# avik-pal/LocalRegNeuralDE.jl

Measured on NVIDIA B200. Metric: mnist_ode_train_samples_per_s, higher is better.
Workload: dtype tf32x3

## Files before the change

localregneuralde.jl_b200/csrc/lrnde_adjoint.cu:

```cuda
#include "lrnde_adjoint.h"

#include <stdio.h>
#include <stdlib.h>
#include <string.h>

#include <algorithm>

#include "lrnde_fused_dev.cuh"

enum {
  LA_ALPHA = 0,
  LA_S1 = 2,
  LA_DEL = 8,
  LA_CC = 13,
  LA_HH = 18,
  LA_EPS = 23,
  LA_DBT = 29,
  LA_HBB = 30,
  LA_HBT = 31,
  LA_NARR = 32
};

#ifdef LRNDE_UMMA_TRACE
__device__ long long g_adj_trace[1024];
// ... 586 lines not shown
            }
          } else if (g < 4) {
            r = __ldcg(reinterpret_cast<const float4*>(o.Q0 + (size_t)b * LR_ZROW + c4 * 4));
          } else if (o.Q1) {
            r = __ldcg(reinterpret_cast<const float4*>(o.Q1 + (size_t)b * LR_ZROW + c4 * 4));
          }
        }
        dst[g] = r;
      }
    };
    if (niter > 0) load_iter(0, v[0]);
    if (niter > 1) load_iter(1, v[1]);
    for (int it0 = 0; it0 < niter; it0 += 2) {
#pragma unroll
      for (int dd = 0; dd < 2; ++dd) {
        const int it = it0 + dd;
        if (it < niter) {
          const int s = it % NS, ph = (it / NS) & 1;
          uint8_t* stage = smem + (size_t)s * kPaStageBytes;
          const Ops o = ops_of(it);
          mbar_wait(&empty_bar[s], (uint32_t)(ph ^ 1));
#pragma unroll
          for (int g = 0; g < 6; ++g) {
            const int li = tid + (g & 1) * PT;
            const int bl = li >> 5, c4 = li & 31;
            const int grp = c4 >> 3, c32 = (c4 & 7) >> 1, half = c4 & 1, k4 = bl >> 2, r = bl & 3;
            const uint32_t off = (uint32_t)((k4 * 4 + grp) * 512 + r * 128 + ((c32 ^ r) << 5) + half * 16);
            float4 xv = (g >= 4 && !o.Q1) ? v[dd][g - 2] : v[dd][g];
            const float sc = (g < 2) ? 1.0f : ((g < 4) ? o.s0 : o.s1);
            xv.x *= sc; xv.y *= sc; xv.z *= sc; xv.w *= sc;
            float4 hi, lo;
            if (q.passes == 3) {
              hi = make_float4(tf32_rna(xv.x), tf32_rna(xv.y), tf32_rna(xv.z), tf32_rna(xv.w));
              lo = make_float4(tf32_rna(xv.x - hi.x), tf32_rna(xv.y - hi.y), tf32_rna(xv.z - hi.z), tf32_rna(xv.w - hi.w));
            } else { hi = xv; lo = make_float4(0.f, 0.f, 0.f, 0.f); }
            uint8_t* img = stage + (g >> 1) * 32768;
            *reinterpret_cast<float4*>(img + off) = hi;
            *reinterpret_cast<float4*>(img + 16384 + off) = lo;
          }
          if (it + 2 < niter) load_iter(it + 2, v[dd]);
          fence_proxy_async();
          __syncwarp();
          if (lane == 0) mbar_arrive(&full_bar[s]);
        }
      }
    }
    mbar_wait(&done_bar, 0);
    tc_fence_after();
    const int quarter = (warp & 3) * 32;
    const int wgroup = (warp - 2) >> 2;
    const int mrow = quarter + lane;
    const int nacc = (job == 0) ? 4 : 2;
    float* out;
    if (job == 0) out = q.partP + (size_t)split * 4 * 16384;
    else out = (job == 1 ? q.partX : q.partL) + ((size_t)split * q.ntile + tile) * 2 * 16384;
    for (int a = 0; a < nacc; ++a) {
      for (int cb = wgroup; cb < 8; cb += kEpiWarps / 4) {
        float r[16];
        tmem_ld16(tmem_base + ((uint32_t)quarter << 16) + (uint32_t)(a * 128 + cb * 16), r);
        float4* o4 = reinterpret_cast<float4*>(out + (size_t)a * 16384 + (size_t)mrow * 128 + cb * 16);
        if (niter == 0) {
#pragma unroll
          for (int j = 0; j < 16; ++j) r[j] = 0.0f;
        }
#pragma unroll
        for (int j = 0; j < 4; ++j) o4[j] = make_float4(r[4 * j], r[4 * j + 1], r[4 * j + 2], r[4 * j + 3]);
      }
    }
    tc_fence_before();
  }
  __syncthreads();
  if (warp == 1) {
    tc_fence_after();
    asm volatile("tcgen05.dealloc.cta_group::1.sync.aligned.b32 %0, %1;" ::"r"(tmem_base), "r"(512u) : "memory");
  }
}

struct AReduceP {
  SolveDev* S;
  const float* partP; const float* partX; const float* partL;
  float* RP; float* RX; float* RL;
  int nP, nD, ntile;
};
__global__ void __launch_bounds__(256) adj_reduce_kernel(AReduceP p) {
  if (p.S->done) return;
  const size_t nP4 = 4 * 4096, nX4 = (size_t)p.ntile * 2 * 4096;
  for (size_t i = blockIdx.x * (size_t)blockDim.x + threadIdx.x; i < nP4 + 2 * nX4; i += (size_t)gridDim.x * blockDim.x) {
    float4 s = make_float4(0.f, 0.f, 0.f, 0.f);
    if (i < nP4) {
      const float4* src = reinterpret_cast<const float4*>(p.partP) + i;
#pragma unroll 8
      for (int k = 0; k < p.nP; ++k) {
        const float4 v = __ldcg(src + (size_t)k * nP4);
        s.x += v.x; s.y += v.y; s.z += v.z; s.w += v.w;
      }
      reinterpret_cast<float4*>(p.RP)[i] = s;
    } else {
      const bool isx = (i - nP4) < nX4;
      const size_t j = isx ? (i - nP4) : (i - nP4 - nX4);
      const float4* src = reinterpret_cast<const float4*>(isx ? p.partX : p.partL) + j;
      for (int k = 0; k < p.nD; ++k) {
        const float4 v = __ldcg(src + (size_t)k * nX4);
        s.x += v.x; s.y += v.y; s.z += v.z; s.w += v.w;
      }
      const size_t tile = j / (2 * 4096), rem = j % (2 * 4096), vv = rem / 4096, mn = rem % 4096;
      float4* dst = reinterpret_cast<float4*>(isx ? p.RX : p.RL);
      dst[(vv * p.ntile + tile) * 4096 + mn] = s;
    }
  }
}

struct AMuP {
  SolveDev* S;
  const float* RP; const float* RX; const float* RL;
  const float* W2a;
  const float* W1T;
  int D, H, td, Kaug, ntile;
  long w1_off, w2_off;
  long nparams;
};
__global__ void __launch_bounds__(512) adj_mu_kernel(AMuP p) {
  SolveDev* S = p.S;
  if (S->done) return;
  const int slot = S->slot, next = (S->slot + 1) % S->cap;
  const float* mu_n = lr_slot_u(S, slot) + S->lam_len;
  float* mu_new = lr_slot_u(S, next) + S->lam_len;
  const float dt = S->err.scale, abstol = S->abstol, reltol = S->reltol;
  const int H = p.H, D = p.D, Kaug = p.Kaug;
  const long n1 = (long)H * (D + p.td + 1), n2 = (long)D * Kaug;
  const size_t RXs = (size_t)p.ntile * 128 * 128;
  const bool multi = S->reduce_mu && S->nranks > 1;
  const int par = (int)(S->mseq & 1ull);
  float* st0 = multi ? lr_mbox_stage(S->mbox[S->rank], par, 0) : nullptr;
  float* st1 = multi ? lr_mbox_stage(S->mbox[S->rank], par, 1) : nullptr;
  double acc = 0.0;
  for (long i = blockIdx.x * (long)blockDim.x + threadIdx.x; i < n1 + n2; i += (long)gridDim.x * blockDim.x) {
    float g0, g1;
    long pidx;
    if (i < n1) {
      const int d = (int)(i / H), r = (int)(i % H);
      pidx = p.w1_off + i;
      if (d < D) {
        float a0 = p.RX[(size_t)d * 128 + r], a1 = p.RX[RXs + (size_t)d * 128 + r];
        const float* w = p.W2a + d;
        const float* P0 = p.RP + r;
        const float* P1 = p.RP + 16384 + r;
#pragma unroll 8
        for (int k = 0; k < Kaug; ++k) {
          const float wv = __ldg(w + (size_t)k * D);
          a0 = fmaf(P0[k * 128], wv, a0);
          a1 = fmaf(P1[k * 128], wv, a1);
        }
        g0 = a0; g1 = a1;
      } else {
        const int krow = (p.td && d == D) ? Kaug : Kaug + 1;
        g0 = p.RP[(size_t)krow * 128 + r];
        g1 = p.RP[16384 + (size_t)krow * 128 + r];
      }
    } else {
      const long i2 = i - n1;
      const int k = (int)(i2 / D), d = (int)(i2 % D);
      pidx = p.w2_off + i2;
      float a0 = 0.0f, a1 = 0.0f;
      const float* P0 = p.RP + 2 * 16384 + (size_t)k * 128;
      const float* P1 = p.RP + 3 * 16384 + (size_t)k * 128;
      const float* w = p.W1T + d;
#pragma unroll 8
      for (int r = 0; r < H; ++r) {
        const float wv = __ldg(w + (size_t)r * D);
        a0 = fmaf(P0[r], wv, a0);
        a1 = fmaf(P1[r], wv, a1);
      }
      g0 = fmaf(-dt, a0, p.RL[(size_t)d * 128 + k]);
      g1 = fmaf(-dt, a1, p.RL[RXs + (size_t)d * 128 + k]);
    }
    if (multi) {
      st0[pidx] = g0;
      st1[pidx] = g1;
      continue;
    }
    const float mn = mu_n[pidx];
    const float mv = fmaf(-dt, g0, mn);
    mu_new[pidx] = mv;
    const float ut = -dt * g1;
    const float r = ut / (abstol + fmaxf(fabsf(mn), fabsf(mv)) * reltol);
    acc += (double)(r * r);
  }
  if (multi) {
    __threadfence_system();
    __syncthreads();
    if (threadIdx.x == 0) {
      const unsigned int prev = atomicAdd(S->mucounter, 1u);
      if (prev == gridDim.x - 1) {
        *S->mucounter = 0;
        __threadfence_system();
        for (int r = 0; r < S->nranks; ++r) {
          volatile unsigned long long* f = &S->mbox[r]->mflag[par][S->rank];
          *f = S->mseq + 1;
        }
      }
    }
    return;
  }
  __shared__ double sh[16];
  for (int o = 16; o > 0; o >>= 1) acc += __shfl_down_sync(0xffffffffu, acc, o);
  if ((threadIdx.x & 31) == 0) sh[threadIdx.x >> 5] = acc;
  __syncthreads();
  if (threadIdx.x == 0) {
    double s = 0.0;
    for (int w = 0; w < (int)(blockDim.x >> 5); ++w) s += sh[w];
    S->partials[LR_ERR_BLOCKS + blockIdx.x] = s;
  }
}

__global__ void __launch_bounds__(256) adj_mu_finish_kernel(SolveDev* S) {
  if (S->done) return;
  const int par = (int)(S->mseq & 1ull);
  LrMailbox* mine = S->mbox[S->rank];
  if (threadIdx.x == 0) {
    long long spins = 0;
    for (int r = 0; r < S->nranks; ++r) {
      volatile unsigned long long* f = &mine->mflag[par][r];
      while (*f != S->mseq + 1) {
        __nanosleep(40);
        if (++spins > (1ll << 26)) { lr_peer_timeout(S); break; }
      }
    }
    __threadfence_system();
  }
  __syncthreads();
  const int slot = S->slot, next = (S->slot + 1) % S->cap;
  const size_t P = S->mu_len;
  const float* mu_n = lr_slot_u(S, slot) + S->lam_len;
  float* mu_new = lr_slot_u(S, next) + S->lam_len;
  const float* mg_n = S->muglob + (size_t)slot * P;
  float* mg_new = S->muglob + (size_t)next * P;
  const float* own0 = lr_mbox_stage(mine, par, 0);
  const float dt = S->err.scale, abstol = S->abstol, reltol = S->reltol;
  double acc = 0.0;
  for (size_t i = blockIdx.x * (size_t)blockDim.x + threadIdx.x; i < P; i += (size_t)gridDim.x * blockDim.x) {
    float g0 = 0.0f, g1 = 0.0f;
    for (int r = 0; r < S->nranks; ++r) {
      g0 += ((const volatile float*)lr_mbox_stage(S->mbox[r], par, 0))[i];
      g1 += ((const volatile float*)lr_mbox_stage(S->mbox[r], par, 1))[i];
    }
    mu_new[i] = fmaf(-dt, ((const volatile float*)own0)[i], mu_n[i]);
    const float mn = mg_n[i];
    const float mv = fmaf(-dt, g0, mn);
    mg_new[i] = mv;
    const float ut = -dt * g1;
    const float rr = ut / (abstol + fmaxf(fabsf(mn), fabsf(mv)) * reltol);
    acc += (double)(rr * rr);
  }
  __shared__ double sh[8];
  for (int o = 16; o > 0; o >>= 1) acc += __shfl_down_sync(0xffffffffu, acc, o);
  if ((threadIdx.x & 31) == 0) sh[threadIdx.x >> 5] = acc;
  __syncthreads();
  if (threadIdx.x == 0) {
    double s = 0.0;
    for (int w = 0; w < 8; ++w) s += sh[w];
    S->partials[LR_ERR_BLOCKS + blockIdx.x] = s;
  }
}

}

#define LRA_COUNT(ctx) do { if ((ctx)->capturing) (ctx)->captured++; else (ctx)->launches++; } while (0)

bool LatentAdjoint::eligible(const lrnde_model* m) {
  FusedShape s;
  if (!lrf_shape(m, &s)) return false;
  return s.KS <= 14 && s.Kaug + 2 <= 128;
}

LatentAdjoint::LatentAdjoint(lrnde_ctx* c, const lrnde_model* mm, const float* p, int64_t b, int npasses)
    : ctx(c), m(mm), ps(p), B(b), passes(npasses) {
  lrf_shape(m, &sh);
  ntiles = (int)((B + fused::kNT - 1) / fused::kNT);
  zlen = (size_t)LR_ZROW * (size_t)ntiles * fused::kNT;
  nunits = (int)((B + 15) / 16);
  unit_bytes = (size_t)sh.nfull * 8192 + (size_t)sh.ntail * 2048;
  const int maxc = std::max(1, 148 / sh.n_mt);
  const int rounds = (nunits + maxc - 1) / maxc;
  nclusters = (nunits + rounds - 1) / rounds;
  ntile_d = (sh.D + 127) / 128;
  const int nchunk_tot = (int)((B + 31) / 32);
  const double wP = 13.0, wD = 2.0 * ntile_d;
  int wantP = std::max(1, (int)(148.0 * wP / (wP + wD)));
  int cP = std::max(1, (nchunk_tot + wantP - 1) / wantP);
  chunkP = cP * 32;
  nP = (int)((B + chunkP - 1) / chunkP);
  int wantD = std::max(1, (148 - nP) / (2 * ntile_d));
  int cD = std::max(1, (nchunk_tot + wantD - 1) / wantD);
  chunkD = cD * 32;
  nD = (int)((B + chunkD - 1) / chunkD);
  Mz = (float*)ctx->alloc(sizeof(float) * 128 * 128);
  ws = (float*)ctx->alloc(sizeof(float) * LA_NARR * zlen);
  alpha_in = (float*)ctx->alloc(sizeof(float) * zlen);
  hbuf = (float*)ctx->alloc((size_t)ntiles * 4 * unit_bytes);
  partP = (float*)ctx->alloc(sizeof(float) * (size_t)nP * 4 * 16384);
  partX = (float*)ctx->alloc(sizeof(float) * (size_t)nD * ntile_d * 2 * 16384);
  partL = (float*)ctx->alloc(sizeof(float) * (size_t)nD * ntile_d * 2 * 16384);
  RP = (float*)ctx->alloc(sizeof(float) * 4 * 16384);
  RX = (float*)ctx->alloc(sizeof(float) * (size_t)ntile_d * 2 * 16384);
  RL = (float*)ctx->alloc(sizeof(float) * (size_t)ntile_d * 2 * 16384);
  static bool attr_set = false;
  if (!attr_set) {
    constexpr int kChainSmem = 4 * (3 * 8192 + 3 * 2048) + ladj::kTapeBufs * ladj::kTapeBufBytes + 1024;
    LR_CUDA(cudaFuncSetAttribute(ladj::adj_chain_kernel<ACT_IDENTITY, false>, cudaFuncAttributeMaxDynamicSharedMemorySize, kChainSmem));
    LR_CUDA(cudaFuncSetAttribute(ladj::adj_chain_kernel<ACT_IDENTITY, true>, cudaFuncAttributeMaxDynamicSharedMemorySize, kChainSmem));
    LR_CUDA(cudaFuncSetAttribute(ladj::adj_chain_kernel<ACT_TANH, false>, cudaFuncAttributeMaxDynamicSharedMemorySize, kChainSmem));
    LR_CUDA(cudaFuncSetAttribute(ladj::adj_chain_kernel<ACT_TANH, true>, cudaFuncAttributeMaxDynamicSharedMemorySize, kChainSmem));
    LR_CUDA(cudaFuncSetAttribute(ladj::adj_chain_kernel<ACT_GELU, false>, cudaFuncAttributeMaxDynamicSharedMemorySize, kChainSmem));
    LR_CUDA(cudaFuncSetAttribute(ladj::adj_chain_kernel<ACT_GELU, true>, cudaFuncAttributeMaxDynamicSharedMemorySize, kChainSmem));
    LR_CUDA(cudaFuncSetAttribute(ladj::adj_chain_kernel<ACT_SIGMOID, false>, cudaFuncAttributeMaxDynamicSharedMemorySize, kChainSmem));
    LR_CUDA(cudaFuncSetAttribute(ladj::adj_chain_kernel<ACT_SIGMOID, true>, cudaFuncAttributeMaxDynamicSharedMemorySize, kChainSmem));
    LR_CUDA(cudaFuncSetAttribute(ladj::adj_chain_kernel<ACT_RELU, false>, cudaFuncAttributeMaxDynamicSharedMemorySize, kChainSmem));
    LR_CUDA(cudaFuncSetAttribute(ladj::adj_chain_kernel<ACT_RELU, true>, cudaFuncAttributeMaxDynamicSharedMemorySize, kChainSmem));
    LR_CUDA(cudaFuncSetAttribute(ladj::pairacc_kernel, cudaFuncAttributeMaxDynamicSharedMemorySize, ladj::pairacc_smem()));
    attr_set = true;
  }
  if (getenv("LRNDE_FUSED_VERBOSE"))
    fprintf(stderr, "[lrnde adjoint] B=%lld tiles=%d units=%d kgemm clusters=%d pairacc: nP=%d x %d samples, nD=%d x %d samples x %d tiles\n",
            (long long)B, ntiles, nunits, nclusters, nP, chunkP, nD, chunkD, ntile_d);
}

LatentAdjoint::~LatentAdjoint() {
  ctx->release(Mz); ctx->release(ws); ctx->release(alpha_in); ctx->release(hbuf);
  ctx->release(partP); ctx->release(partX); ctx->release(partL);
  ctx->release(RP); ctx->release(RX); ctx->release(RL);
}

void LatentAdjoint::prepare(const float* mz_plain) {
  if (mz_plain) { Mz_ext = mz_plain; return; }
  lrf_mz_plain(ctx, m, ps, Mz);
  LRA_COUNT(ctx);
}

static void lra_launch_chain(LatentAdjoint& E, SolveDev* S, int single) {
  const FusedShape& sh = E.sh;
  const LayerInfo& L1 = E.m->layers[0];
  ladj::AChainP cp;
  memset(&cp, 0, sizeof(cp));
  cp.S = S; cp.single = single; cp.Mz = E.Mz_ext ? E.Mz_ext : E.Mz;
  cp.w1t = sh.td ? E.ps + L1.w_off + (size_t)sh.D * sh.H : nullptr;
  cp.b1 = E.ps + L1.b_off;
  cp.Zx = E.Zx; cp.alpha_in = E.alpha_in; cp.ws = E.ws; cp.zlen = E.zlen;
  cp.hbuf = E.hbuf; cp.unit_bytes = (uint32_t)E.unit_bytes;
  cp.B = (int)E.B; cp.H = sh.H; cp.td = sh.td; cp.Kaug = sh.Kaug; cp.KS = sh.KS; cp.nfull = sh.nfull; cp.ntail = sh.ntail;
  cp.passes = E.passes;
  const size_t smem_c = 4 * ((size_t)sh.nfull * 8192 + (size_t)sh.ntail * 2048) + ladj::kTapeBufs * ladj::kTapeBufBytes + 1024;
  cudaStream_t st = E.ctx->stream;
#define LRA_CHAIN(A) do { if (single) ladj::adj_chain_kernel<A, true><<<E.ntiles, fused::kThreads, smem_c, st>>>(cp); \
                         else ladj::adj_chain_kernel<A, false><<<E.ntiles, fused::kThreads, smem_c, st>>>(cp); } while (0)
  switch (sh.act) {
    case ACT_TANH: LRA_CHAIN(ACT_TANH); break;
    case ACT_GELU: LRA_CHAIN(ACT_GELU); break;
    case ACT_SIGMOID: LRA_CHAIN(ACT_SIGMOID); break;
    case ACT_RELU: LRA_CHAIN(ACT_RELU); break;
    default: LRA_CHAIN(ACT_IDENTITY); break;
  }
#undef LRA_CHAIN
  LRA_COUNT(E.ctx);
  LR_CUDA(cudaGetLastError());
}

static void lra_launch_pairacc(LatentAdjoint& E, SolveDev* S) {
  ladj::PairAccP q;
  memset(&q, 0, sizeof(q));
  q.S = S; q.ws = E.ws; q.zlen = E.zlen; q.x = E.x; q.D = E.sh.D; q.B = (int)E.B;
  q.nP = E.nP; q.chunkP = E.chunkP; q.nD = E.nD; q.chunkD = E.chunkD; q.ntile = E.ntile_d;
  q.partP = E.partP; q.partX = E.partX; q.partL = E.partL; q.passes = E.passes;
  int n = 0;
  for (int j = 1; j <= 7; ++j) {
    const float bj = (j <= 6) ? lr_tsit5_a(5, j - 1) : 0.0f;
    const float btj = lr_tsit5_btilde(j - 1);
    const int del = (j == 1) ? -1 : ((j == 7) ? -10 : LA_DEL + j - 2);
    const int hh = (j == 1) ? -2 : ((j == 7) ? -11 : LA_HH + j - 2);
    const int cc = (j == 1) ? -3 : ((j == 7) ? -12 : LA_CC + j - 2);
    q.term[n++] = {cc, del, bj, btj, 0};
    if (j >= 2) q.term[n++] = {hh, LA_EPS + j - 2, bj, btj, 1};
  }
  q.nterm = n;
  const int grid = E.nP + 2 * E.ntile_d * E.nD;
  ladj::pairacc_kernel<<<grid, fused::kThreads, ladj::pairacc_smem(), E.ctx->stream>>>(q);
  LRA_COUNT(E.ctx);
  LR_CUDA(cudaGetLastError());
}

static void lra_launch_mu(LatentAdjoint& E, SolveDev* S) {
  cudaStream_t st = E.ctx->stream;
  ladj::AReduceP r;
  r.S = S; r.partP = E.partP; r.partX = E.partX; r.partL = E.partL; r.RP = E.RP; r.RX = E.RX; r.RL = E.RL;
  r.nP = E.nP; r.nD = E.nD; r.ntile = E.ntile_d;
  const size_t n4 = 4 * 4096 + 2 * (size_t)E.ntile_d * 2 * 4096;
  ladj::adj_reduce_kernel<<<(int)((n4 + 255) / 256), 256, 0, st>>>(r);
  LRA_COUNT(E.ctx);
  const LayerInfo& L1 = E.m->layers[0];
  const LayerInfo& L2 = E.m->layers[1];
  ladj::AMuP mp;
  memset(&mp, 0, sizeof(mp));
  mp.S = S; mp.RP = E.RP; mp.RX = E.RX; mp.RL = E.RL;
  mp.W2a = E.ps + L2.w_off; mp.W1T = E.W1T;
  mp.D = E.sh.D; mp.H = E.sh.H; mp.td = E.sh.td; mp.Kaug = E.sh.Kaug; mp.ntile = E.ntile_d;
  mp.w1_off = (long)L1.w_off; mp.w2_off = (long)L2.w_off; mp.nparams = (long)E.m->nparams;
  ladj::adj_mu_kernel<<<LR_ERR_BLOCKS, 512, 0, st>>>(mp);
  LRA_COUNT(E.ctx);
  if (E.ctx->nranks > 1) {
    ladj::adj_mu_finish_kernel<<<LR_ERR_BLOCKS, 256, 0, st>>>(S);
    LRA_COUNT(E.ctx);
  }
  LR_CUDA(cudaGetLastError());
}

void LatentAdjoint::begin(SolveDev* S) { lra_launch_chain(*this, S, 1); }

void LatentAdjoint::attempt(SolveDev* S) {
  lra_launch_chain(*this, S, 0);
  lrf_launch_kgemm_adj(ctx, S, sh, ps + m->layers[0].w_off, hbuf, unit_bytes, B, passes, nunits, nclusters);
  lra_launch_pairacc(*this, S);
  lra_launch_mu(*this, S);
}

void LatentAdjoint::attempt_part(SolveDev* S, int which) {
  if (which == 0) lra_launch_chain(*this, S, 0);
  else if (which == 1) lrf_launch_kgemm_adj(ctx, S, sh, ps + m->layers[0].w_off, hbuf, unit_bytes, B, passes, nunits, nclusters);
  else if (which == 2) lra_launch_pairacc(*this, S);
  else lra_launch_mu(*this, S);
}
```

localregneuralde.jl_b200/csrc/lrnde_api.cu:

```cuda
#include <stdarg.h>
#include <stdio.h>
#include <stdlib.h>
#include <string.h>

#include <algorithm>
#include <chrono>
#include <cmath>
#include <functional>
#include <memory>

#include "lrnde_host.h"
#include "lrnde_kernels.cuh"
#include "lrnde_umma.cuh"
#include "lrnde_smem_mlp.cuh"
#include "lrnde_conv.cuh"
#include "lrnde_conv_tc.h"
#include "lrnde_fused.h"
#include "lrnde_adjoint.h"
#include "lrnde_regrev.cuh"

static bool lr_reg_hidden_eligible(const lrnde_model* m, int reg_type);

static thread_local char g_err[1024] = "";
void lr_set_error(const char* fmt, ...) {
// ... 1222 lines not shown
    h.abstol = abstol;
    h.reltol = reltol;
    h.slot = 0;
    h.done = 0;
    h.failed = 0;
    h.tape_full = 0;
  }

  void body_signature(std::vector<lrnde_ctx::GraphNodeSig>& sig) {
    cudaStream_t st = ctx->stream;
    cudaGraph_t probe = nullptr;
    ctx->capturing = true;
    const long before = ctx->captured;
    cudaError_t e = cudaStreamBeginCapture(st, cudaStreamCaptureModeThreadLocal);
    if (e != cudaSuccess) { ctx->capturing = false; LR_CUDA(e); }
    try { body(); } catch (...) {
      cudaGraph_t dummy; cudaStreamEndCapture(st, &dummy); ctx->capturing = false; ctx->captured = before; throw;
    }
    e = cudaStreamEndCapture(st, &probe);
    ctx->capturing = false;
    ctx->captured = before;
    LR_CUDA(e);
    size_t n = 0;
    LR_CUDA(cudaGraphGetNodes(probe, nullptr, &n));
    std::vector<cudaGraphNode_t> nodes(n);
    if (n) LR_CUDA(cudaGraphGetNodes(probe, nodes.data(), &n));
    sig.clear();
    bool ok = true;
    for (size_t i = 0; i < n && ok; ++i) {
      cudaGraphNodeType ty;
      LR_CUDA(cudaGraphNodeGetType(nodes[i], &ty));
      if (ty != cudaGraphNodeTypeKernel) { ok = false; break; }
      cudaKernelNodeParams kp;
      LR_CUDA(cudaGraphKernelNodeGetParams(nodes[i], &kp));
      lrnde_ctx::GraphNodeSig s;
      s.func = kp.func;
      s.g[0] = kp.gridDim.x; s.g[1] = kp.gridDim.y; s.g[2] = kp.gridDim.z;
      s.b[0] = kp.blockDim.x; s.b[1] = kp.blockDim.y; s.b[2] = kp.blockDim.z;
      s.smem = kp.sharedMemBytes;
      if (!kp.kernelParams) { ok = false; break; }
      for (size_t pi = 0;; ++pi) {
        size_t off = 0, sz = 0;
        if (cudaFuncGetParamInfo(kp.func, pi, &off, &sz) != cudaSuccess) { cudaGetLastError(); break; }
        const char* src = (const char*)kp.kernelParams[pi];
        s.params.insert(s.params.end(), src, src + sz);
      }
      sig.push_back(std::move(s));
    }
    cudaGraphDestroy(probe);
    if (!ok) sig.clear();
  }

  void build_graphs(int loop_mode) {
    cudaStream_t st = ctx->stream;
    if (loop_mode == 0) {
      std::vector<lrnde_ctx::GraphNodeSig> sig;
      const bool use_cache = getenv("LRNDE_NO_GRAPH_CACHE") == nullptr;
      if (use_cache) {
        body_signature(sig);
        for (auto& cg : ctx->graph_cache) {
          if (cg.dev != (void*)dev || cg.sig.size() != sig.size()) continue;
          bool same = true;
          for (size_t i = 0; i < sig.size() && same; ++i) {
            const auto &a = cg.sig[i], &b = sig[i];
            same = a.func == b.func && memcmp(a.g, b.g, sizeof(a.g)) == 0 && memcmp(a.b, b.b, sizeof(a.b)) == 0 &&
                   a.smem == b.smem && a.params == b.params;
          }
          if (!same) continue;
          while_graph = cg.graph; while_exec = cg.exec; graph_cached = true;
          h.cond_handle = cg.handle; h.use_cond = 1; body_nodes = cg.body_nodes;
          cg.last_use = ++ctx->graph_clock;
          return;
        }
      }
      LR_CUDA(cudaGraphCreate(&while_graph, 0));
      cudaGraphConditionalHandle handle;
      LR_CUDA(cudaGraphConditionalHandleCreate(&handle, while_graph, 0, 0));
      h.cond_handle = (unsigned long long)handle;
      h.use_cond = 1;
      cudaGraphNode_t prime;
      cudaKernelNodeParams kp;
      memset(&kp, 0, sizeof(kp));
      SolveDev* d = dev;
      void* args[] = {&d};
      kp.func = (void*)cond_prime_kernel_entry();
      kp.gridDim = dim3(1);
      kp.blockDim = dim3(32);
      kp.kernelParams = args;
      LR_CUDA(cudaGraphAddKernelNode(&prime, while_graph, nullptr, 0, &kp));
      cudaGraphNodeParams cp = {cudaGraphNodeTypeConditional};
      cp.type = cudaGraphNodeTypeConditional;
      cp.conditional.handle = handle;
      cp.conditional.type = cudaGraphCondTypeWhile;
      cp.conditional.size = 1;
      cudaGraphNode_t cond;
      LR_CUDA(cudaGraphAddNode(&cond, while_graph, &prime, 1, &cp));
      cudaGraph_t bodyg = cp.conditional.phGraph_out[0];
      ctx->capturing = true;
      long before = ctx->captured;
      cudaError_t e = cudaStreamBeginCaptureToGraph(st, bodyg, nullptr, nullptr, 0,
                                                    cudaStreamCaptureModeThreadLocal);
      if (e != cudaSuccess) { ctx->capturing = false; LR_CUDA(e); }
      try { body(); } catch (...) {
        cudaGraph_t dummy; cudaStreamEndCapture(st, &dummy); ctx->capturing = false; throw;
      }
      cudaGraph_t outg = nullptr;
      e = cudaStreamEndCapture(st, &outg);
      ctx->capturing = false;
      LR_CUDA(e);
      body_nodes = ctx->captured - before;
      LR_CUDA(cudaGraphInstantiate(&while_exec, while_graph, 0));
      if (use_cache && !sig.empty()) {
        if (ctx->graph_cache.size() >= 8) {
          size_t lru = 0;
          for (size_t i = 1; i < ctx->graph_cache.size(); ++i)
            if (ctx->graph_cache[i].last_use < ctx->graph_cache[lru].last_use) lru = i;
          cudaGraphExecDestroy(ctx->graph_cache[lru].exec);
          cudaGraphDestroy(ctx->graph_cache[lru].graph);
          ctx->graph_cache.erase(ctx->graph_cache.begin() + lru);
        }
        lrnde_ctx::CachedGraph cg;
        cg.graph = while_graph; cg.exec = while_exec; cg.handle = h.cond_handle; cg.body_nodes = body_nodes;
        cg.dev = (void*)dev; cg.sig = std::move(sig); cg.last_use = ++ctx->graph_clock;
        ctx->graph_cache.push_back(std::move(cg));
        graph_cached = true;
      }
    } else if (loop_mode == 2) {
      h.use_cond = 0;
      long before = ctx->launches;
      (void)before;
      body_nodes = 0;
    } else {
      h.use_cond = 0;
      ctx->capturing = true;
      long before = ctx->captured;
      cudaError_t e = cudaStreamBeginCapture(st, cudaStreamCaptureModeThreadLocal);
      if (e != cudaSuccess) { ctx->capturing = false; LR_CUDA(e); }
      try { body(); } catch (...) {
        cudaGraph_t dummy; cudaStreamEndCapture(st, &dummy); ctx->capturing = false; throw;
      }
      e = cudaStreamEndCapture(st, &body_graph);
      ctx->capturing = false;
      LR_CUDA(e);
      body_nodes = ctx->captured - before;
      LR_CUDA(cudaGraphInstantiate(&body_exec, body_graph, 0));
    }
  }
  static void* cond_prime_kernel_entry();

  void run_segment() {
    cudaStream_t st = ctx->stream;
    if (while_exec) {
      LR_CUDA(cudaGraphLaunch(while_exec, st));
      ctx->launches += 1;
    } else {
      int* pin = (int*)((char*)ctx->pinned + sizeof(SolveDev) + 64);
      for (;;) {
        for (int i = 0; i < 8; ++i) {
          if (body_exec) LR_CUDA(cudaGraphLaunch(body_exec, st));
          else body();
        }
        LR_CUDA(cudaMemcpyAsync(pin, &dev->done, sizeof(int), cudaMemcpyDeviceToHost, st));
        LR_CUDA(cudaStreamSynchronize(st));
        if (*pin) break;
      }
    }
  }
};

__global__ void cond_prime_kernel(SolveDev* S) {
  if (threadIdx.x == 0) lr_set_cond(S);
}
void* Solver::cond_prime_kernel_entry() { return (void*)cond_prime_kernel; }

struct lrnde_tape {
  lrnde_ctx* ctx;
  const lrnde_model* model;
  lrnde_opts opts;
  int64_t B;
  float* ps = nullptr;
  float* bn_state = nullptr;
  float* Mz = nullptr;
  int reg_hidden = 0;
  std::unique_ptr<Solver> fwd;
  std::unique_ptr<Solver> reg;
  std::vector<float> fts;
  std::vector<float> save_ts;
  std::vector<int> save_out;
  int reg_mode = 0;
  int lean = 0;
  float t1 = 0.f;
  std::vector<float> log_t[2], log_dt[2], log_eest[2];
  std::vector<unsigned char> log_acc[2];
  ~lrnde_tape() { ctx->release(ps); ctx->release(bn_state); ctx->release(Mz); }
};

static void lr_copy_log(Solver& S, lrnde_tape* T, int which) {
  int n = std::min(S.h.nlog, S.h.logcap);
  T->log_t[which].resize(n);
  T->log_dt[which].resize(n);
  T->log_eest[which].resize(n);
  T->log_acc[which].resize(n);
  if (n == 0) return;
  cudaStream_t st = S.ctx->stream;
  LR_CUDA(cudaMemcpyAsync(T->log_t[which].data(), S.h.log_t, 4 * (size_t)n, cudaMemcpyDeviceToHost, st));
  LR_CUDA(cudaMemcpyAsync(T->log_dt[which].data(), S.h.log_dt, 4 * (size_t)n, cudaMemcpyDeviceToHost, st));
  LR_CUDA(cudaMemcpyAsync(T->log_eest[which].data(), S.h.log_eest, 4 * (size_t)n, cudaMemcpyDeviceToHost, st));
  LR_CUDA(cudaMemcpyAsync(T->log_acc[which].data(), S.h.log_acc, (size_t)n, cudaMemcpyDeviceToHost, st));
  LR_CUDA(cudaStreamSynchronize(st));
}

static void lr_mu_exchange(Solver& S, int mode, int nvec, const int* done) {
  if (!(S.h.reduce_mu && S.h.nranks > 1)) return;
  lrnde_ctx* ctx = S.ctx;
  cudaStream_t st = ctx->stream;
  mu_publish_kernel<<<64, 256, 0, st>>>(S.dev, mode, done);
  LR_COUNT(ctx);
  mu_gather_kernel<<<64, 256, 0, st>>>(S.dev, nvec, done);
  LR_COUNT(ctx);
  mu_norm_kernel<<<LR_ERR_BLOCKS, 256, 0, st>>>(S.dev, mode, done);
  LR_COUNT(ctx);
}

template <class EvalFn>
static void lr_solver_start(Solver& S, EvalFn&& eval, int begin) {
  lrnde_ctx* ctx = S.ctx;
  cudaStream_t st = ctx->stream;
  k1_desc_kernel<<<1, 32, 0, st>>>(S.dev);
  LR_COUNT(ctx);
  eval(&S.dev->st[6], &S.dev->yint[6], &S.dev->failed, nullptr, false);
  initdt_norm1_kernel<<<LR_ERR_BLOCKS, 256, 0, st>>>(S.dev);
  LR_COUNT(ctx);
  lr_mu_exchange(S, 0, 1, &S.dev->failed);
  initdt_a_kernel<<<1, 32, 0, st>>>(S.dev);
  LR_COUNT(ctx);
  eval(&S.dev->st[0], &S.dev->yint[1], &S.dev->failed, nullptr, false);
  initdt_norm2_kernel<<<LR_ERR_BLOCKS, 256, 0, st>>>(S.dev);
  LR_COUNT(ctx);
  lr_mu_exchange(S, 1, 1, &S.dev->failed);
  initdt_b_kernel<<<1, 32, 0, st>>>(S.dev, begin);
  LR_COUNT(ctx);
  LR_CHECK_LAUNCH();
}

template <class EvalFn>
static void lr_step_body(Solver& S, EvalFn&& eval, bool fuse_unew = false) {
  lrnde_ctx* ctx = S.ctx;
  cudaStream_t st = ctx->stream;
  for (int j = 0; j < 5; ++j) eval(&S.dev->st[j], &S.dev->yint[j + 1], &S.dev->done, nullptr, false);
  if (fuse_unew) {
    eval(&S.dev->st[5], &S.dev->yint[6], &S.dev->done, &S.dev->st[6], true);
  } else {
    lincomb_kernel<<<lr_ew_blocks(S.h.len), 256, 0, st>>>(&S.dev->st[5], nullptr, S.h.len, &S.dev->done);
    LR_COUNT(ctx);
// ... 700 lines not shown
  if (nsteps >= 1) {
    const bool timing = getenv("LRNDE_TIMING") != nullptr;
    long tmark = lr_now_us();
    auto mark = [&](const char* what) {
      if (!timing) return;
      cudaStreamSynchronize(st);
      const long now = lr_now_us();
      fprintf(stderr, "[lrnde] bwd %-14s %8ld us\n", what, now - tmark);
      tmark = now;
    };
    Solver A(ctx, len, DB, 2, 1, o.maxiters + 1);
    mark("solver alloc");
    A.h.is_adjoint = 1;
    A.h.fts = F.ts;
    A.h.ftape = F.tape;
    A.h.flen = DB;
    A.h.fnsteps = nsteps;
    A.h.ftdir = 1;
    std::unique_ptr<LatentAdjoint> la;
    if (T->lean && getenv("LRNDE_NO_LATENT_ADJ"))
      lr_fail(LRNDE_ESTATE, "the forward solve kept a lean tape (latent-space adjoint); set LRNDE_FULL_TAPE=1 for the forward to use the per-layer adjoint");
    if (F.htape && ev.use_umma && LatentAdjoint::eligible(m) && !getenv("LRNDE_NO_LATENT_ADJ")) {
      la = std::make_unique<LatentAdjoint>(ctx, m, T->ps, B, ev.passes);
      la->W1T = ev.WT[0]; la->Zx = F.ztape; la->x = F.tape;
      la->prepare(T->Mz);
      A.h.fhtape = F.htape;
      A.h.fztape = F.ztape;
      A.h.fzlen = F.h.zlen;
      A.h.lat_mu_row = 1;
    }
    auto latent_begin = [&]() {
      const LayerInfo& L2 = m->layers[1];
      DenseP p;
      memset(&p, 0, sizeof(p));
      p.A = ev.WT[1]; p.lda = L2.in; p.M = L2.in; p.K = L2.out; p.td = 0; p.bias = 0;
      p.xdesc = &A.dev->cur; p.ldx = L2.out; p.N = (int)B;
      p.Y = la->alpha_in; p.ldy = LR_ZROW; p.act = ACT_IDENTITY; p.dact = -1; p.out_scale = 1.0f;
      p.done = &A.dev->failed;
      ev.dense(p, ev.packWT[1]);
      la->begin(A.dev);
    };
    if (ctx->nranks > 1) {
      A.h.total_len = (unsigned long long)D * (unsigned long long)ctx->total_batch + P;
      A.enable_mu_exchange(P);
    }
    std::vector<float> stops;
    for (float s : T->save_ts) {
      float sc = std::min(s, t2);
      if (sc > t0 && sc < t2 && std::find(stops.begin(), stops.end(), sc) == stops.end()) stops.push_back(sc);
    }
    std::sort(stops.begin(), stops.end(), [](float a, float b) { return a > b; });
    stops.push_back(t0);
    A.init_ctrl(t2, t0, stops[0], o.maxiters, o.pow_mode, o.abstol, o.reltol);
    std::unique_ptr<FusedEngine> fe_y;
    std::unique_ptr<DevBuf> ybuf, ydescs;
    if (T->lean) {
      if (!la) lr_fail(LRNDE_ESTATE, "lean forward tape but the latent-space adjoint is not available for this call");
      fe_y = std::make_unique<FusedEngine>(ctx, m, T->ps, B, ev.passes);
      ybuf = std::make_unique<DevBuf>(ctx, DB);
      ydescs = std::make_unique<DevBuf>(ctx, 2 * (sizeof(LinComb) / 4 + 1));
      LinComb od;
      memset(&od, 0, sizeof(od));
      od.dst = ybuf->p;
      LR_CUDA(cudaMemcpyAsync(ydescs->p, &od, sizeof(LinComb), cudaMemcpyHostToDevice, st));
    }
    auto rhs = [&](const LinComb* in, const LinComb* y, const int* done, const LinComb*, bool) {
      if (T->lean) {
        LinComb* out_desc = (LinComb*)ydescs->p;
        LinComb* y_mat = out_desc + 1;
        fe_y->dense_output_dev(A.dev, y, F.tape, ybuf->p, y_mat, out_desc);
        y = y_mat;
      }
      ev.vjp(y, in, nullptr, in, -1.0f, nullptr, in, DB, -1.0f, 0.0f, done);
    };
    A.body = [&]() {
      if (la) {
        la->attempt(A.dev);
        controller_kernel<<<1, 32, 0, st>>>(A.dev);
        LR_COUNT(ctx);
        LR_CHECK_LAUNCH();
      } else lr_step_body(A, rhs);
    };
    mark("latent setup");
    A.build_graphs(o.loop_mode);
    A.upload();
    mark("graphs");
    LR_CUDA(cudaMemsetAsync(A.tape, 0, sizeof(float) * len, st));
    std::vector<const float*> blocks;
    cot_blocks(t2, blocks);
    for (auto b : blocks) {
      axpy_kernel<<<lr_ew_blocks(DB), 256, 0, st>>>(A.tape, b, 1.0f, DB);
      LR_COUNT(ctx);
    }
    lr_solver_start(A, rhs, 1);
    mark("solver start");
    if (la && A.muglob) LR_CUDA(cudaMemsetAsync(A.muglob, 0, sizeof(float) * P, st));
    if (la) latent_begin();
    mark("latent begin");
    if (la && getenv("LRNDE_PROFILE_ADJ")) {
      const int iters = std::max(1, atoi(getenv("LRNDE_PROFILE_ADJ")));
      cudaEvent_t e[6];
      for (auto& ev_ : e) LR_CUDA(cudaEventCreate(&ev_));
      for (int w = 0; w < 2; ++w) la->attempt(A.dev);
      for (int k = 0; k < 4; ++k) {
        LR_CUDA(cudaEventRecord(e[k], st));
        for (int i = 0; i < iters; ++i) la->attempt_part(A.dev, k);
      }
      LR_CUDA(cudaEventRecord(e[4], st));
      for (int i = 0; i < iters; ++i) la->attempt(A.dev);
      LR_CUDA(cudaEventRecord(e[5], st));
      LR_CUDA(cudaEventSynchronize(e[5]));
      const char* nm[5] = {"chain", "lambda gemm", "pairacc", "reduce + mu", "attempt"};
      for (int k = 0; k < 5; ++k) {
        float ms = 0.0f;
        LR_CUDA(cudaEventElapsedTime(&ms, e[k], e[k + 1]));
        g_adj_profile_us[k] = 1000.0f * ms / (float)iters;
        if (timing) fprintf(stderr, "[lrnde] adjoint attempt: %-12s %8.1f us\n", nm[k], g_adj_profile_us[k]);
      }
      for (auto& ev_ : e) cudaEventDestroy(ev_);
    }
    for (size_t si = 0; si < stops.size(); ++si) {
      A.run_segment();
      mark("segment");
      if (si + 1 < stops.size()) {
        cot_blocks(stops[si], blocks);
        for (auto b : blocks) {
          jump_kernel<<<lr_ew_blocks(DB), 256, 0, st>>>(A.dev, b, DB);
          LR_COUNT(ctx);
        }
        k1_desc_kernel<<<1, 32, 0, st>>>(A.dev);
        LR_COUNT(ctx);
        if (la) latent_begin();
        else rhs(&A.dev->st[6], &A.dev->yint[6], &A.dev->failed, nullptr, false);
        segment_begin_kernel<<<1, 32, 0, st>>>(A.dev, stops[si + 1], 1);
        LR_COUNT(ctx);
        nbwd_stops++;
      }
    }
    LR_CHECK_LAUNCH();
    A.download();
    lr_copy_log(A, T, 1);
    const float* z = A.tape + (size_t)A.h.slot * 7 * len;
    LR_CUDA(cudaMemcpyAsync(dx_dev, z, sizeof(float) * DB, cudaMemcpyDeviceToDevice, st));
    LR_CUDA(cudaMemcpyAsync(dps_dev, z + DB, sizeof(float) * P, cudaMemcpyDeviceToDevice, st));
    cot_blocks(t0, blocks);
    for (auto b : blocks) {
      axpy_kernel<<<lr_ew_blocks(DB), 256, 0, st>>>(dx_dev, b, 1.0f, DB);
      LR_COUNT(ctx);
    }
    retcode_bwd = A.h.c.retcode;
    nacc_b = A.h.c.naccept;
    nrej_b = A.h.c.nreject;
    body_launches = A.body_nodes * (long)A.h.nlog;
    LR_CUDA(cudaStreamSynchronize(st));
  } else {
    LR_CUDA(cudaMemsetAsync(dx_dev, 0, sizeof(float) * DB, st));
    LR_CUDA(cudaMemsetAsync(dps_dev, 0, sizeof(float) * P, st));
  }

  const long tb_adj = lr_now_us();
  if (T->reg && d_reg != 0.0f && T->reg_hidden && ev.use_umma && !getenv("LRNDE_NO_HIDDEN_REG")) {
    lr_reg_pullback_hidden(ctx, m, T, ev, d_reg, dps_dev);
  } else if (T->reg && d_reg != 0.0f) {
    Solver& R = *T->reg;
    DevBuf work(ctx, 9 * DB);
    RegSeedP sp;
    sp.R = R.dev; sp.reg_type = o.reg_type; sp.d_reg = d_reg;
    for (int k = 0; k < 6; ++k) sp.dk[k] = work.p + (size_t)k * DB;
    sp.du = work.p + 6 * DB;
    sp.dg6 = work.p + 7 * DB;
    float* abuf = work.p + 8 * DB;
    reg_seed_kernel<<<lr_ew_blocks(DB), 256, 0, st>>>(sp);
    LR_COUNT(ctx);
    std::vector<LinComb> lam(6);
    for (int k = 0; k < 6; ++k) { memset(&lam[k], 0, sizeof(LinComb)); lam[k].base = sp.dk[k]; }
    DevBuf dl(ctx, 6 * (sizeof(LinComb) / 4 + 1));
    LR_CUDA(cudaMemcpyAsync(dl.p, lam.data(), sizeof(LinComb) * 6, cudaMemcpyHostToDevice, st));
    const LinComb* lamd = (const LinComb*)dl.p;
    for (int row = 5; row >= 0; --row) {
      const LinComb* y = (row == 5) ? &R.dev->st[6] : &R.dev->st[row];
      ev.vjp(y, lamd + row, abuf, nullptr, 1.0f, dps_dev, nullptr, 0, 1.0f, 1.0f, nullptr);
// ... 186 lines not shown
```

Measured before the change: 1.079 million.

## Tile adjoint mu kernel with shared-memory staging and register blocking

Rewrites the adjoint mu-gradient kernel so each block handles tiles. The reduced partial products and weights are staged in shared memory, and each thread accumulates four outputs in registers instead of reading global memory in a per-element dot loop. The reduce kernel's block size shrinks and its unroll factor grows. Separately, the while-graph conditional prime now writes the handle and cond flag itself, and graph building moves after latent setup. This adds dynamic shared memory and tile-bound logic, and it changes graph capture ordering.

```diff
diff --git a/localregneuralde.jl_b200/csrc/lrnde_adjoint.cu b/localregneuralde.jl_b200/csrc/lrnde_adjoint.cu
--- a/localregneuralde.jl_b200/csrc/lrnde_adjoint.cu
+++ b/localregneuralde.jl_b200/csrc/lrnde_adjoint.cu
@@ -692,14 +692,15 @@
   float* RP; float* RX; float* RL;
   int nP, nD, ntile;
 };
-__global__ void __launch_bounds__(256) adj_reduce_kernel(AReduceP p) {
+constexpr int kReduceThreads = 64;
+__global__ void __launch_bounds__(kReduceThreads) adj_reduce_kernel(AReduceP p) {
   if (p.S->done) return;
   const size_t nP4 = 4 * 4096, nX4 = (size_t)p.ntile * 2 * 4096;
   for (size_t i = blockIdx.x * (size_t)blockDim.x + threadIdx.x; i < nP4 + 2 * nX4; i += (size_t)gridDim.x * blockDim.x) {
     float4 s = make_float4(0.f, 0.f, 0.f, 0.f);
     if (i < nP4) {
       const float4* src = reinterpret_cast<const float4*>(p.partP) + i;
-#pragma unroll 8
+#pragma unroll 16
       for (int k = 0; k < p.nP; ++k) {
         const float4 v = __ldcg(src + (size_t)k * nP4);
         s.x += v.x; s.y += v.y; s.z += v.z; s.w += v.w;
@@ -729,65 +730,36 @@
   long w1_off, w2_off;
   long nparams;
 };
-__global__ void __launch_bounds__(512) adj_mu_kernel(AMuP p) {
+constexpr int kMuThreads = 256;
+constexpr int kMuT1 = 8;
+constexpr int kMuT2d = 64, kMuT2k = 16;
+constexpr int kMuL = kMuT2k + 1;
+__host__ __device__ constexpr size_t mu_smem_w1(int Kaug) { return sizeof(float) * (2 * (size_t)(Kaug + 2) * 128 + (size_t)Kaug * kMuT1); }
+__host__ __device__ constexpr size_t mu_smem_w2(int H) {
+  return sizeof(float) * (2 * (size_t)H * kMuT2k + (size_t)H * kMuT2d + 2 * (size_t)kMuT2d * kMuL);
+}
+__global__ void __launch_bounds__(kMuThreads) adj_mu_kernel(AMuP p) {
   SolveDev* S = p.S;
   if (S->done) return;
+  extern __shared__ float4 mu_smem4[];
+  float* sm = reinterpret_cast<float*>(mu_smem4);
+  const int tid = threadIdx.x;
   const int slot = S->slot, next = (S->slot + 1) % S->cap;
   const float* mu_n = lr_slot_u(S, slot) + S->lam_len;
   float* mu_new = lr_slot_u(S, next) + S->lam_len;
   const float dt = S->err.scale, abstol = S->abstol, reltol = S->reltol;
   const int H = p.H, D = p.D, Kaug = p.Kaug;
-  const long n1 = (long)H * (D + p.td + 1), n2 = (long)D * Kaug;
   const size_t RXs = (size_t)p.ntile * 128 * 128;
   const bool multi = S->reduce_mu && S->nranks > 1;
   const int par = (int)(S->mseq & 1ull);
   float* st0 = multi ? lr_mbox_stage(S->mbox[S->rank], par, 0) : nullptr;
   float* st1 = multi ? lr_mbox_stage(S->mbox[S->rank], par, 1) : nullptr;
   double acc = 0.0;
-  for (long i = blockIdx.x * (long)blockDim.x + threadIdx.x; i < n1 + n2; i += (long)gridDim.x * blockDim.x) {
-    float g0, g1;
-    long pidx;
-    if (i < n1) {
-      const int d = (int)(i / H), r = (int)(i % H);
-      pidx = p.w1_off + i;
-      if (d < D) {
-        float a0 = p.RX[(size_t)d * 128 + r], a1 = p.RX[RXs + (size_t)d * 128 + r];
-        const float* w = p.W2a + d;
-        const float* P0 = p.RP + r;
-        const float* P1 = p.RP + 16384 + r;
-#pragma unroll 8
-        for (int k = 0; k < Kaug; ++k) {
-          const float wv = __ldg(w + (size_t)k * D);
-          a0 = fmaf(P0[k * 128], wv, a0);
-          a1 = fmaf(P1[k * 128], wv, a1);
-        }
-        g0 = a0; g1 = a1;
-      } else {
-        const int krow = (p.td && d == D) ? Kaug : Kaug + 1;
-        g0 = p.RP[(size_t)krow * 128 + r];
-        g1 = p.RP[16384 + (size_t)krow * 128 + r];
-      }
-    } else {
-      const long i2 = i - n1;
-      const int k = (int)(i2 / D), d = (int)(i2 % D);
-      pidx = p.w2_off + i2;
-      float a0 = 0.0f, a1 = 0.0f;
-      const float* P0 = p.RP + 2 * 16384 + (size_t)k * 128;
-      const float* P1 = p.RP + 3 * 16384 + (size_t)k * 128;
-      const float* w = p.W1T + d;
-#pragma unroll 8
-      for (int r = 0; r < H; ++r) {
-        const float wv = __ldg(w + (size_t)r * D);
-        a0 = fmaf(P0[r], wv, a0);
-        a1 = fmaf(P1[r], wv, a1);
-      }
-      g0 = fmaf(-dt, a0, p.RL[(size_t)d * 128 + k]);
-      g1 = fmaf(-dt, a1, p.RL[RXs + (size_t)d * 128 + k]);
-    }
+  auto emit = [&](long pidx, float g0, float g1) {
     if (multi) {
       st0[pidx] = g0;
       st1[pidx] = g1;
-      continue;
+      return;
     }
     const float mn = mu_n[pidx];
     const float mv = fmaf(-dt, g0, mn);
@@ -795,6 +767,94 @@
     const float ut = -dt * g1;
     const float r = ut / (abstol + fmaxf(fabsf(mn), fabsf(mv)) * reltol);
     acc += (double)(r * r);
+  };
+  const int nt1 = (D + p.td + 1 + kMuT1 - 1) / kMuT1;
+  const int nk2 = (Kaug + kMuT2k - 1) / kMuT2k;
+  const int nt = nt1 + nk2 * ((D + kMuT2d - 1) / kMuT2d);
+  for (int t = blockIdx.x; t < nt; t += gridDim.x) {
+    __syncthreads();
+    if (t < nt1) {
+      const int d0 = t * kMuT1, KR = Kaug + 2;
+      float* Ps = sm;
+      float* Ws = sm + 2 * (size_t)KR * 128;
+      for (int i = tid; i < 2 * KR * 32; i += kMuThreads) {
+        const int v = i / (KR * 32), rem = i % (KR * 32);
+        reinterpret_cast<float4*>(Ps)[i] = __ldcg(reinterpret_cast<const float4*>(p.RP + (size_t)v * 16384) + rem);
+      }
+      for (int i = tid; i < Kaug * kMuT1; i += kMuThreads) {
+        const int k = i / kMuT1, d = d0 + i % kMuT1;
+        Ws[i] = (d < D) ? __ldg(p.W2a + (size_t)k * D + d) : 0.0f;
+      }
+      __syncthreads();
+      const int r = tid & 127, jq = tid >> 7, c0 = d0 + jq * 4;
+      if (r < H) {
+        float a0[4], a1[4];
+#pragma unroll
+        for (int j = 0; j < 4; ++j) {
+          const int d = c0 + j;
+          a0[j] = (d < D) ? p.RX[(size_t)d * 128 + r] : 0.0f;
+          a1[j] = (d < D) ? p.RX[RXs + (size_t)d * 128 + r] : 0.0f;
+        }
+        const float* P0 = Ps + r;
+        const float* P1 = Ps + (size_t)KR * 128 + r;
+        const float4* W4 = reinterpret_cast<const float4*>(Ws) + jq;
+#pragma unroll 4
+        for (int k = 0; k < Kaug; ++k) {
+          const float4 w = W4[k * (kMuT1 / 4)];
+          const float x0 = P0[k * 128], x1 = P1[k * 128];
+          a0[0] = fmaf(x0, w.x, a0[0]); a0[1] = fmaf(x0, w.y, a0[1]); a0[2] = fmaf(x0, w.z, a0[2]); a0[3] = fmaf(x0, w.w, a0[3]);
+          a1[0] = fmaf(x1, w.x, a1[0]); a1[1] = fmaf(x1, w.y, a1[1]); a1[2] = fmaf(x1, w.z, a1[2]); a1[3] = fmaf(x1, w.w, a1[3]);
+        }
+#pragma unroll
+        for (int j = 0; j < 4; ++j) {
+          const int d = c0 + j;
+          if (d < D) emit(p.w1_off + (long)d * H + r, a0[j], a1[j]);
+          else if (d < D + p.td + 1) {
+            const int krow = (p.td && d == D) ? Kaug : Kaug + 1;
+            emit(p.w1_off + (long)d * H + r, P0[krow * 128], P1[krow * 128]);
+          }
+        }
+      }
+    } else {
+      const int t2 = t - nt1, k0 = (t2 % nk2) * kMuT2k, d0 = (t2 / nk2) * kMuT2d;
+      float* Xs = sm;
+      float* Ys = Xs + 2 * (size_t)H * kMuT2k;
+      float* Ls = Ys + (size_t)H * kMuT2d;
+      for (int i = tid; i < 2 * kMuT2k * H; i += kMuThreads) {
+        const int v = i / (kMuT2k * H), rem = i % (kMuT2k * H), kl = rem / H, r = rem % H;
+        Xs[((size_t)v * H + r) * kMuT2k + kl] = (k0 + kl < Kaug) ? __ldcg(p.RP + (size_t)(2 + v) * 16384 + (size_t)(k0 + kl) * 128 + r) : 0.0f;
+      }
+      for (int i = tid; i < H * kMuT2d; i += kMuThreads) {
+        const int r = i / kMuT2d, d = d0 + i % kMuT2d;
+        Ys[i] = (d < D) ? __ldg(p.W1T + (size_t)r * D + d) : 0.0f;
+      }
+      for (int i = tid; i < 2 * kMuT2d * kMuT2k; i += kMuThreads) {
+        const int v = i / (kMuT2d * kMuT2k), rem = i % (kMuT2d * kMuT2k), dl = rem / kMuT2k, kl = rem % kMuT2k;
+        const int d = d0 + dl, k = k0 + kl;
+        Ls[((size_t)v * kMuT2d + dl) * kMuL + kl] = (d < D && k < Kaug) ? __ldcg(p.RL + v * RXs + (size_t)d * 128 + k) : 0.0f;
+      }
+      __syncthreads();
+      const int dl = tid % kMuT2d, kq = tid / kMuT2d, d = d0 + dl;
+      float a0[4] = {0.0f, 0.0f, 0.0f, 0.0f}, a1[4] = {0.0f, 0.0f, 0.0f, 0.0f};
+      const float4* X0 = reinterpret_cast<const float4*>(Xs) + kq;
+      const float4* X1 = reinterpret_cast<const float4*>(Xs + (size_t)H * kMuT2k) + kq;
+#pragma unroll 4
+      for (int r = 0; r < H; ++r) {
+        const float y = Ys[r * kMuT2d + dl];
+        const float4 x0 = X0[r * (kMuT2k / 4)], x1 = X1[r * (kMuT2k / 4)];
+        a0[0] = fmaf(x0.x, y, a0[0]); a0[1] = fmaf(x0.y, y, a0[1]); a0[2] = fmaf(x0.z, y, a0[2]); a0[3] = fmaf(x0.w, y, a0[3]);
+        a1[0] = fmaf(x1.x, y, a1[0]); a1[1] = fmaf(x1.y, y, a1[1]); a1[2] = fmaf(x1.z, y, a1[2]); a1[3] = fmaf(x1.w, y, a1[3]);
+      }
+      if (d < D) {
+#pragma unroll
+        for (int j = 0; j < 4; ++j) {
+          const int kl = kq * 4 + j, k = k0 + kl;
+          if (k < Kaug)
+            emit(p.w2_off + (long)k * D + d, fmaf(-dt, a0[j], Ls[(size_t)dl * kMuL + kl]),
+                 fmaf(-dt, a1[j], Ls[((size_t)kMuT2d + dl) * kMuL + kl]));
+        }
+      }
+    }
   }
   if (multi) {
     __threadfence_system();
@@ -812,13 +872,13 @@
     }
     return;
   }
-  __shared__ double sh[16];
+  __shared__ double sh[kMuThreads / 32];
   for (int o = 16; o > 0; o >>= 1) acc += __shfl_down_sync(0xffffffffu, acc, o);
   if ((threadIdx.x & 31) == 0) sh[threadIdx.x >> 5] = acc;
   __syncthreads();
   if (threadIdx.x == 0) {
     double s = 0.0;
-    for (int w = 0; w < (int)(blockDim.x >> 5); ++w) s += sh[w];
+    for (int w = 0; w < kMuThreads / 32; ++w) s += sh[w];
     S->partials[LR_ERR_BLOCKS + blockIdx.x] = s;
   }
 }
@@ -928,6 +988,8 @@
     LR_CUDA(cudaFuncSetAttribute(ladj::adj_chain_kernel<ACT_RELU, false>, cudaFuncAttributeMaxDynamicSharedMemorySize, kChainSmem));
     LR_CUDA(cudaFuncSetAttribute(ladj::adj_chain_kernel<ACT_RELU, true>, cudaFuncAttributeMaxDynamicSharedMemorySize, kChainSmem));
     LR_CUDA(cudaFuncSetAttribute(ladj::pairacc_kernel, cudaFuncAttributeMaxDynamicSharedMemorySize, ladj::pairacc_smem()));
+    LR_CUDA(cudaFuncSetAttribute(ladj::adj_mu_kernel, cudaFuncAttributeMaxDynamicSharedMemorySize,
+                                 (int)std::max(ladj::mu_smem_w1(126), ladj::mu_smem_w2(126))));
     attr_set = true;
   }
   if (getenv("LRNDE_FUSED_VERBOSE"))
@@ -1004,7 +1066,7 @@
   r.S = S; r.partP = E.partP; r.partX = E.partX; r.partL = E.partL; r.RP = E.RP; r.RX = E.RX; r.RL = E.RL;
   r.nP = E.nP; r.nD = E.nD; r.ntile = E.ntile_d;
   const size_t n4 = 4 * 4096 + 2 * (size_t)E.ntile_d * 2 * 4096;
-  ladj::adj_reduce_kernel<<<(int)((n4 + 255) / 256), 256, 0, st>>>(r);
+  ladj::adj_reduce_kernel<<<(int)((n4 + ladj::kReduceThreads - 1) / ladj::kReduceThreads), ladj::kReduceThreads, 0, st>>>(r);
   LRA_COUNT(E.ctx);
   const LayerInfo& L1 = E.m->layers[0];
   const LayerInfo& L2 = E.m->layers[1];
@@ -1014,7 +1076,8 @@
   mp.W2a = E.ps + L2.w_off; mp.W1T = E.W1T;
   mp.D = E.sh.D; mp.H = E.sh.H; mp.td = E.sh.td; mp.Kaug = E.sh.Kaug; mp.ntile = E.ntile_d;
   mp.w1_off = (long)L1.w_off; mp.w2_off = (long)L2.w_off; mp.nparams = (long)E.m->nparams;
-  ladj::adj_mu_kernel<<<LR_ERR_BLOCKS, 512, 0, st>>>(mp);
+  const size_t smem = std::max(ladj::mu_smem_w1(E.sh.Kaug), ladj::mu_smem_w2(E.sh.H));
+  ladj::adj_mu_kernel<<<LR_ERR_BLOCKS, ladj::kMuThreads, smem, st>>>(mp);
   LRA_COUNT(E.ctx);
   if (E.ctx->nranks > 1) {
     ladj::adj_mu_finish_kernel<<<LR_ERR_BLOCKS, 256, 0, st>>>(S);
diff --git a/localregneuralde.jl_b200/csrc/lrnde_api.cu b/localregneuralde.jl_b200/csrc/lrnde_api.cu
--- a/localregneuralde.jl_b200/csrc/lrnde_api.cu
+++ b/localregneuralde.jl_b200/csrc/lrnde_api.cu
@@ -1328,7 +1328,8 @@
       cudaKernelNodeParams kp;
       memset(&kp, 0, sizeof(kp));
       SolveDev* d = dev;
-      void* args[] = {&d};
+      unsigned long long hd = h.cond_handle;
+      void* args[] = {&d, &hd};
       kp.func = (void*)cond_prime_kernel_entry();
       kp.gridDim = dim3(1);
       kp.blockDim = dim3(32);
@@ -1414,8 +1415,12 @@
   }
 };
 
-__global__ void cond_prime_kernel(SolveDev* S) {
-  if (threadIdx.x == 0) lr_set_cond(S);
+__global__ void cond_prime_kernel(SolveDev* S, unsigned long long handle) {
+  if (threadIdx.x == 0) {
+    S->cond_handle = handle;
+    S->use_cond = 1;
+    lr_set_cond(S);
+  }
 }
 void* Solver::cond_prime_kernel_entry() { return (void*)cond_prime_kernel; }
 
@@ -2282,9 +2287,7 @@
       } else lr_step_body(A, rhs);
     };
     mark("latent setup");
-    A.build_graphs(o.loop_mode);
     A.upload();
-    mark("graphs");
     LR_CUDA(cudaMemsetAsync(A.tape, 0, sizeof(float) * len, st));
     std::vector<const float*> blocks;
     cot_blocks(t2, blocks);
@@ -2297,6 +2300,8 @@
     if (la && A.muglob) LR_CUDA(cudaMemsetAsync(A.muglob, 0, sizeof(float) * P, st));
     if (la) latent_begin();
     mark("latent begin");
+    A.build_graphs(o.loop_mode);
+    mark("graphs");
     if (la && getenv("LRNDE_PROFILE_ADJ")) {
       const int iters = std::max(1, atoi(getenv("LRNDE_PROFILE_ADJ")));
       cudaEvent_t e[6];
```

Result: faster. 1.107 million, median of 6 (+2.6%).
